# CAMMA-public/SelfPose3d

Measured on AMD Instinct MI355X. Metric: multi-view samples/sec (5-view Panoptic, 80x80x20 voxel), higher is better.
Workload: dtype f32

## Files before the change

selfpose3d_amd/build.py:

```python
from __future__ import annotations

import os
import subprocess
import sys

HERE = os.path.dirname(os.path.abspath(__file__))
CSRC = os.path.join(HERE, "csrc")
SOURCES = ["sp3d_unproject.hip", "sp3d_proposal.hip", "sp3d_epilogue.hip", "sp3d_upconv.hip", "sp3d_synth.hip", "sp3d_fftconv.hip", "sp3d_wino.hip",
           "sp3d_wino_fused.hip", "sp3d_conv3_direct.hip", "sp3d_fft.hip", "sp3d_gbn.hip"]
HEADERS = [os.path.join("..", "pk_src1.py"), "sp3d_conv3_host.h", "sp3d_device.h", "sp3d_proj_pk.h", "sp3d_split.h", "sp3d_tuning.h",
           "sp3d_twiddles.h", os.path.join("..", "..", "include", "sp3d.h")]
LIB = os.path.join(HERE, "libsp3d.so")
HIPCC = os.environ.get("HIPCC", "/opt/rocm/bin/hipcc")
FLAGS = ["--offload-arch=gfx950", "-O3", "-std=c++17", "-ffp-contract=off", "-munsafe-fp-atomics", "-fPIC", "-shared",
         "-Wall", "-Wno-unused-function"]
LINK = ["-L/opt/rocm/lib", "-lhipfft"]


def needs_build() -> bool:
    if not os.path.exists(LIB):
        return True
    t = os.path.getmtime(LIB)
    deps = [os.path.join(CSRC, s) for s in SOURCES + HEADERS] + [os.path.abspath(__file__)]
    return any(os.path.getmtime(d) > t for d in deps if os.path.exists(d))


PER_SOURCE_FLAGS = {"sp3d_wino.hip": ["-fno-slp-vectorize"], "sp3d_wino_fused.hip": ["-fno-slp-vectorize"],
                    "sp3d_conv3_direct.hip": ["-fno-slp-vectorize"], "sp3d_upconv.hip": ["-fno-slp-vectorize"],
                    "sp3d_fft.hip": ["-fno-slp-vectorize"], "sp3d_fftconv.hip": ["-fno-slp-vectorize"]}


LLVM_BIN = os.environ.get("SP3D_LLVM_BIN", "/opt/rocm/lib/llvm/bin")

NOPK_LIB = os.path.join(HERE, "libsp3d_nopk.so")
NOPK_FLAGS = ["-DSP3D_NO_PK", "-fno-slp-vectorize", "-Xclang", "-target-feature", "-Xclang", "-packed-fp32-ops"]




def _compile_one(src: str, objdir: str, cflags, verbose: bool, host_flags=()) -> str:
    from . import pk_src1
    base = os.path.join(objdir, src.replace(".hip", ""))
    path = os.path.join(CSRC, src)
    cuid = "-cuid=" + src.replace(".", "_")

    def run(cmd):
        if verbose:
            print(" ".join(cmd))
        subprocess.check_call(cmd)
    if os.environ.get("SP3D_PLAIN_HIPCC", "0") not in ("", "0"):
        flags = cflags + [f for f in NOPK_FLAGS if f not in cflags]
        run([HIPCC] + flags + ["-Wno-unused-command-line-argument", "-c", path, "-o", base + ".o"])
        return base + ".o"
    run([HIPCC] + cflags + ["-Wno-unused-command-line-argument", "--cuda-device-only", "-S", cuid, path, "-o", base + ".raw.s"])
    try:
        with open(base + ".raw.s") as fh:
            text, n = pk_src1.fix_asm(fh.read())
    except ValueError as e:
        import warnings
        warnings.warn(f"{src}: {e}; compiling this source without packed-fp32 instructions")
        cflags = cflags + [f for f in NOPK_FLAGS if f not in cflags]
        run([HIPCC] + cflags + ["-Wno-unused-command-line-argument", "--cuda-device-only", "-S", cuid, path, "-o", base + ".raw.s"])
        with open(base + ".raw.s") as fh:
            text, n = pk_src1.fix_asm(fh.read())
    if pk_src1.count_risky(text):
        raise RuntimeError(f"{src}: packed-fp32 instructions reading the high half of source 1 survive the rewrite")
    with open(base + ".s", "w") as fh:
        fh.write(text)
    os.remove(base + ".raw.s")
    if verbose:
        print(f"{src}: {n} packed-fp32 instructions rewritten (source 0 <-> source 1)")
    run([os.path.join(LLVM_BIN, "clang"), "-x", "assembler", "-target", "amdgcn-amd-amdhsa", "-mcpu=gfx950", "-c", base + ".s", "-o", base + ".dev.o"])
    run([os.path.join(LLVM_BIN, "lld"), "-flavor", "gnu", "-m", "elf64_amdgpu", "--no-undefined", "-shared", "-o", base + ".hsaco", base + ".dev.o"])
    run([os.path.join(LLVM_BIN, "clang-offload-bundler"), "-type=o", "-bundle-align=4096",
         "-targets=host-x86_64-unknown-linux-gnu,hipv4-amdgcn-amd-amdhsa--gfx950", "-input=/dev/null", "-input=" + base + ".hsaco",
         "-output=" + base + ".hipfb"])
    run([HIPCC] + cflags + list(host_flags) + ["-Wno-unused-command-line-argument", "--cuda-host-only", cuid, "-Xclang",
                                               "-fcuda-include-gpubinary", "-Xclang", base + ".hipfb", "-c", path, "-o", base + ".o"])
    for ext in (".dev.o", ".hsaco", ".hipfb"):
        os.remove(base + ext)
    return base + ".o"


def _compile_objects(objdir: str, extra_flags=(), verbose: bool = False, host_flags=()):
    from concurrent.futures import ThreadPoolExecutor
    os.makedirs(objdir, exist_ok=True)
    cflags = [f for f in FLAGS if f != "-shared"]
    with ThreadPoolExecutor(max_workers=len(SOURCES)) as pool:
        futs = [pool.submit(_compile_one, src, objdir, cflags + list(extra_flags) + PER_SOURCE_FLAGS.get(src, []), verbose, host_flags)
                for src in SOURCES]
        return [f.result() for f in futs]


def _link(objs, out: str, verbose: bool = False, link_flags=()):
    cmd = [HIPCC, "--offload-arch=gfx950", "-shared", "-fPIC"] + objs + LINK + list(link_flags) + ["-o", out]
    if verbose:
        print(" ".join(cmd))
    subprocess.check_call(cmd)


def build_variant(out: str, extra_flags=(), host_flags=(), link_flags=()) -> str:
    objdir = out + ".obj"
    _link(_compile_objects(objdir, extra_flags, host_flags=host_flags), out, link_flags=link_flags)
    return out


def _stale(lib: str) -> bool:
    if not os.path.exists(lib):
        return True
    t = os.path.getmtime(lib)
    deps = [os.path.join(CSRC, s) for s in SOURCES + HEADERS] + [os.path.abspath(__file__)]
    return any(os.path.getmtime(d) > t for d in deps if os.path.exists(d))


def build(force: bool = False, verbose: bool = False) -> str:
    if force or needs_build():
        objs = _compile_objects(os.path.join(HERE, "build", "obj"), verbose=verbose)
        _link(objs, LIB + ".tmp", verbose)
        os.replace(LIB + ".tmp", LIB)
    if force or _stale(NOPK_LIB):
        objs = _compile_objects(os.path.join(HERE, "build", "obj_nopk"), NOPK_FLAGS, verbose=verbose)
        _link(objs, NOPK_LIB + ".tmp", verbose)
        os.replace(NOPK_LIB + ".tmp", NOPK_LIB)
    return LIB


if __name__ == "__main__":
    print(build(force="--force" in sys.argv, verbose=True))
```

selfpose3d_amd/csrc/sp3d_conv3_direct.hip:

```cpp
#include <hip/hip_runtime.h>
#include <stdint.h>

#include "../../include/sp3d.h"
#include "sp3d_conv3_host.h"
#include "sp3d_split.h"

namespace sp3d {

constexpr int CD_BX = 16, CD_BY = 8, CD_BZ = 4;
constexpr int CD_RX = CD_BX + 2, CD_RY = CD_BY + 2, CD_RZ = CD_BZ + 2, CD_VOX = 8, CD_ROW = CD_RX * CD_VOX, CD_ZP = CD_RY * CD_ROW + 4;
constexpr int CD_PLANE = CD_RZ * CD_ZP;
constexpr int CD_BUF = 2 * CD_PLANE;
constexpr int CD_NV4 = CD_RX * CD_RY * CD_RZ * 2;
constexpr int CD_PROD = 4;
constexpr int CD_PER = (CD_NV4 + 64 * CD_PROD - 1) / (64 * CD_PROD);
constexpr int CD_BUFS = ((CD_BUF / 4 + 63) / 64) * 256;
#ifndef SP3D_WG_ABLATE
#define SP3D_WG_ABLATE 0
#endif
struct CdRec { u32x4 hl, hh, mm; };


#ifdef SP3D_CD_TIMELINE
__device__ unsigned long long *g_cd_tl = nullptr;
#define CD_STAMP(slot) do { __builtin_amdgcn_sched_barrier(0); if (g_cd_tl && blockIdx.x == 0 && lane == 0 && item < 64) { g_cd_tl[(wave * 64 + item) * 4 + (slot)] = __builtin_readcyclecounter(); \
     \
    if (wave == 0 && (slot) == 0 && item == 0) { g_cd_tl[(7 * 64 + 62) * 4 + 0] = wall_clock64(); g_cd_tl[(7 * 64 + 62) * 4 + 1] = __builtin_readcyclecounter(); } \
    if (wave == 0 && (slot) == 3) { g_cd_tl[(7 * 64 + 63) * 4 + 0] = wall_clock64(); g_cd_tl[(7 * 64 + 63) * 4 + 1] = __builtin_readcyclecounter(); } } __builtin_amdgcn_sched_barrier(0); } while (0)
#else
#define CD_STAMP(slot) do { (void)item; } while (0)
#endif

template <int C, int MODE, bool SKIP = false>
__global__ __launch_bounds__(64 * (4 + CD_PROD)) __attribute__((amdgpu_waves_per_eu(2, 2)))
void conv3_split_kernel(const float *__restrict__ x, const unsigned *__restrict__ W3, float *__restrict__ y,
                        const float *__restrict__ shift, const float *__restrict__ res, int B, int X, int Y, int Z, int NBX,
                        int NBY, int NBZ, int nblocks, const float *__restrict__ xs = nullptr,
                        const unsigned *__restrict__ WS = nullptr)
{
    constexpr int O = 32, NCH = C / 8, CS = 16;
    extern __shared__ __attribute__((aligned(16))) unsigned cd_lds[];
    const int tid = threadIdx.x, lane = tid & 63, wave = tid >> 6, t = lane & 31, h = lane >> 5;
    const int my_blocks = ((int)blockIdx.x < nblocks) ? (nblocks - 1 - (int)blockIdx.x) / (int)gridDim.x + 1 : 0;
    const int n_items = my_blocks * NCH;
    auto decode = [&](int item, int &b, int &ox0, int &oy0, int &oz0) {
        int bid = (int)blockIdx.x + (item / NCH) * (int)gridDim.x;
        const int bz = bid % NBZ; bid /= NBZ;
        const int by = bid % NBY; bid /= NBY;
        const int bx = bid % NBX;
        b = bid / NBX;
        ox0 = bx * CD_BX; oy0 = by * CD_BY; oz0 = bz * CD_BZ;
    };

    if (wave >= 4) {
        const int pt = tid - 256;
        __builtin_amdgcn_s_setprio(2);
        float4 d[CD_PER];
        int lo_[CD_PER], rel[CD_PER], vxyz[CD_PER];
#pragma unroll
        for (int u = 0; u < CD_PER; ++u) {
            const int idx = pt + 64 * CD_PROD * u;
            const int v = idx >> 1, half = idx & 1;
            const int vx = v % CD_RX, vy = (v / CD_RX) % CD_RY, vz = v / (CD_RX * CD_RY);
            lo_[u] = idx < CD_NV4 ? half * CD_PLANE + vz * CD_ZP + vy * CD_ROW + vx * CD_VOX : -1;
            rel[u] = ((vx * Y + vy) * Z + vz) * C + half * 4;
            vxyz[u] = idx < CD_NV4 ? (vx | (vy << 8) | (vz << 16)) : 0x00ffffff;
        }
        auto issue = [&](int k) {
            int b, ox0, oy0, oz0;
            decode(k, b, ox0, oy0, oz0);
            const int64_t vox0 = (((int64_t)b * X + (ox0 - 1)) * Y + (oy0 - 1)) * Z + (oz0 - 1);
            const float *xb = x + vox0 * C + (k % NCH) * 8;
            const int xlo = 1 - ox0, xhi = X + 1 - ox0, ylo = 1 - oy0, yhi = Y + 1 - oy0, zlo = 1 - oz0, zhi = Z + 1 - oz0;
#pragma unroll
            for (int u = 0; u < CD_PER; ++u) {
                const int vx = vxyz[u] & 255, vy = (vxyz[u] >> 8) & 255, vz = vxyz[u] >> 16;
                const bool in = vx >= xlo && vx < xhi && vy >= ylo && vy < yhi && vz >= zlo && vz < zhi;
                d[u] = make_float4(0.0f, 0.0f, 0.0f, 0.0f);
                if (in) d[u] = *reinterpret_cast<const float4 *>(xb + rel[u]);
            }
        };
        if (n_items > 0) issue(0);
        for (int k = 0; k <= n_items; ++k) {
            if (k < n_items) {
                { const int item = k; CD_STAMP(0); }
                unsigned *buf = cd_lds + (k & 1) * CD_BUFS;
#ifdef SP3D_CD_TIMELINE
                __builtin_amdgcn_s_waitcnt(0);
                { const int item = k; CD_STAMP(3); }
#endif
#pragma unroll
                for (int u = 0; u < CD_PER; ++u) {
                    u32x4 q0, q1;
                    split3(d[u], q0, q1);
                    if (lo_[u] >= 0) {
                        unsigned *p = buf + lo_[u];
                        *reinterpret_cast<u32x4 *>(p) = q0;
                        *reinterpret_cast<u32x4 *>(p + 4) = q1;
                    }
                }
                { const int item = k; CD_STAMP(1); }
                if (k + 1 < n_items) issue(k + 1);
            }
            if (k < n_items) { const int item = k; CD_STAMP(2); }
            __syncthreads();
        }
        return;
    }

    const int a_off = h * CD_PLANE + (t >> 3) * CD_ZP + (t & 7) * CD_ROW + 4 * wave * CD_VOX;
    const unsigned *wl = W3 + ((int64_t)h * O + t) * 12;
    struct W3Rec { CdRec d[3]; };
    auto load_w = [&](int q) {
        const int cc = (q / 9) % NCH, st = q % 9;
        const unsigned *r = wl + ((int64_t)(3 * st) * NCH + cc) * 2 * O * 12;
        W3Rec w;
#pragma unroll
        for (int dx = 0; dx < 3; ++dx) {
#if SP3D_W16_ABLATE & 2
            (void)r; w.d[dx].hl = u32x4{0x3f803f80u + (unsigned)q, 0x3f803f80u, 0x3f803f80u + (unsigned)dx, 0x3f803f80u};
            w.d[dx].hh = w.d[dx].hl ^ 0x00010001u; w.d[dx].mm = w.d[dx].hl ^ 0x00020002u;
#else
            w.d[dx].hl = *reinterpret_cast<const u32x4 *>(r + (int64_t)dx * NCH * 2 * O * 12);
            w.d[dx].hh = *reinterpret_cast<const u32x4 *>(r + (int64_t)dx * NCH * 2 * O * 12 + 4);
            w.d[dx].mm = *reinterpret_cast<const u32x4 *>(r + (int64_t)dx * NCH * 2 * O * 12 + 8);
#endif
        }
        return w;
    };
    struct Opnd { u32x4 lh[6], hm[6]; };
    f32x16 acc[4];
    W3Rec w0, w1;
    if (n_items > 0) w0 = load_w(0);
    __syncthreads();
    for (int k = 1; k <= n_items; ++k) {
        const int item = k - 1, cc = item % NCH;
        const unsigned *ab = cd_lds + (item & 1) * CD_BUFS + a_off;
        if (cc == 0) {
#pragma unroll
            for (int m = 0; m < 4; ++m)
#pragma unroll
                for (int v = 0; v < 16; ++v) acc[m][v] = 0.0f;
        }
        auto load_a = [&](int st, Opnd &a) {
            const int dz = st / 3, dy = st % 3;
#pragma unroll
            for (int j = 0; j < 6; ++j) {
                const unsigned *p = ab + dz * CD_ZP + dy * CD_ROW + j * CD_VOX;
                a.lh[j] = *reinterpret_cast<const u32x4 *>(p);
                a.hm[j] = *reinterpret_cast<const u32x4 *>(p + 4);
            }
        };
        Opnd a0, a1;
        load_a(0, a0);
        const int q0 = item * 9;
        float s0[4];
        unsigned so[4];
        CD_STAMP(0);
#pragma unroll
        for (int st = 0; st < 9; ++st) {
            if (SKIP && st == 8 && cc == NCH - 1) {
                int b, ox0, oy0, oz0;
                decode(item, b, ox0, oy0, oz0);
                const float *xb = xs + (int64_t)b * X * Y * Z * CS;
                const int ys = min(oy0 + (t & 7), Y - 1), zs = min(oz0 + (t >> 3), Z - 1);
#pragma unroll
                for (int i = 0; i < 4; ++i) {
                    const int xv = min(ox0 + 4 * wave + i, X - 1);
                    so[i] = (unsigned)(((xv * Y + ys) * Z + zs) * CS + 4 * h);
                    s0[i] = xb[so[i]];
                }
            }
            __builtin_amdgcn_sched_barrier(0);
            w1 = load_w(min(q0 + st + 1, n_items * 9 - 1));
            if (st + 1 < 9) load_a(st + 1, a1);
#pragma unroll
            for (int dx = 0; dx < 3; ++dx) {
#pragma unroll
                for (int i = 0; i < 4; ++i) acc[i] = mfma_bf16(a0.lh[i + dx], w0.d[dx].hl, acc[i]);
#pragma unroll
                for (int i = 0; i < 4; ++i) acc[i] = mfma_bf16(a0.hm[i + dx], w0.d[dx].hh, acc[i]);
#pragma unroll
                for (int i = 0; i < 4; ++i) acc[i] = mfma_bf16(a0.hm[i + dx], w0.d[dx].mm, acc[i]);
            }
#pragma unroll
            for (int r = 0; r < 12; ++r) {
                __builtin_amdgcn_sched_group_barrier(0x008, 1, 0);
                __builtin_amdgcn_sched_group_barrier(0x100, 1, 0);
            }
#pragma unroll
            for (int r = 0; r < 9; ++r) {
                __builtin_amdgcn_sched_group_barrier(0x008, 1, 0);
                __builtin_amdgcn_sched_group_barrier(0x020, 1, 0);
            }
            __builtin_amdgcn_sched_group_barrier(0x008, 15, 0);
            __builtin_amdgcn_sched_barrier(0);
            a0 = a1;
            w0 = w1;
        }
        CD_STAMP(1);
        if (SKIP && cc == NCH - 1) {
            float4 sv[2][4];
            {
                int b, ox0, oy0, oz0;
                decode(item, b, ox0, oy0, oz0);
                const float *xb = xs + (int64_t)b * X * Y * Z * CS;
#pragma unroll
                for (int i = 0; i < 4; ++i) {
                    const float *p = xb + so[i];
                    sv[0][i] = make_float4(s0[i], p[1], p[2], p[3]);
                    sv[1][i] = *reinterpret_cast<const float4 *>(p + 8);
                }
            }
            CdRec ws[2];
#pragma unroll
            for (int c2 = 0; c2 < 2; ++c2) {
                const unsigned *r = WS + (unsigned)(((c2 * 2 + h) * O + t) * 12);
                ws[c2].hl = *reinterpret_cast<const u32x4 *>(r);
                ws[c2].hh = *reinterpret_cast<const u32x4 *>(r + 4);
                ws[c2].mm = *reinterpret_cast<const u32x4 *>(r + 8);
            }
#pragma unroll
            for (int c2 = 0; c2 < 2; ++c2) {
                __builtin_amdgcn_sched_barrier(0);
                u32x4 lh[4], hm[4];
#pragma unroll
                for (int i = 0; i < 4; ++i) split3(sv[c2][i], lh[i], hm[i]);
#pragma unroll
                for (int i = 0; i < 4; ++i) acc[i] = mfma_bf16(lh[i], ws[c2].hl, acc[i]);
#pragma unroll
                for (int i = 0; i < 4; ++i) acc[i] = mfma_bf16(hm[i], ws[c2].hh, acc[i]);
#pragma unroll
                for (int i = 0; i < 4; ++i) acc[i] = mfma_bf16(hm[i], ws[c2].mm, acc[i]);
            }
        }
        if (cc == NCH - 1) {
            int b, ox0, oy0, oz0;
            decode(item, b, ox0, oy0, oz0);
            if (ox0 + CD_BX <= X && oy0 + CD_BY <= Y && oz0 + CD_BZ <= Z) {
                const float sh = shift[t];
                const int64_t obase = ((((int64_t)b * X + ox0 + 4 * wave) * Y + oy0 + 4 * h) * Z + oz0) * O + t;
#pragma unroll
                for (int i = 0; i < 4; ++i)
#pragma unroll
                    for (int v = 0; v < 16; ++v) {
                        const int64_t idx = obase + (((int64_t)i * Y + (v & 3)) * Z + (v >> 2)) * O;
                        float val = acc[i][v] + sh;
                        if (MODE == 2) val += res[idx];
                        if (MODE >= 1) val = SKIP ? relu_keep_nan(val) : fmaxf(val, 0.0f);
                        if (MODE == 3) val += res[idx];
#if SP3D_W16_ABLATE & 16
                        if (val == 123.456f)
#endif
                        y[idx] = val;
                    }
            } else {
            float *scr = reinterpret_cast<float *>(cd_lds + 2 * CD_BUFS) + wave * 1024;
            const int g = lane & 7;
            const float4 sh4 = *reinterpret_cast<const float4 *>(shift + 4 * g);
#pragma unroll
            for (int mb = 0; mb < 4; ++mb) {
#pragma unroll
                for (int v = 0; v < 16; ++v) scr[(8 * (v >> 2) + (v & 3) + 4 * h) * 32 + t] = acc[mb][v];
                __builtin_amdgcn_fence(__ATOMIC_RELEASE, "wavefront");
                __builtin_amdgcn_wave_barrier();
#pragma unroll
                for (int r = 0; r < 4; ++r) {
                    const int m = (lane >> 3) + 8 * r;
                    float4 a = *reinterpret_cast<const float4 *>(scr + m * 32 + 4 * g);
                    const int xo = ox0 + 4 * wave + mb, yo = oy0 + (m & 7), zo = oz0 + (m >> 3);
                    if (xo < X && yo < Y && zo < Z) {
                        const int64_t vox = (((int64_t)b * X + xo) * Y + yo) * Z + zo;
                        a.x += sh4.x; a.y += sh4.y; a.z += sh4.z; a.w += sh4.w;
                        float4 rr = make_float4(0.0f, 0.0f, 0.0f, 0.0f);
                        if (MODE >= 2) rr = *reinterpret_cast<const float4 *>(res + vox * O + 4 * g);
                        if (MODE == 2) { a.x += rr.x; a.y += rr.y; a.z += rr.z; a.w += rr.w; }
                        if (MODE >= 1 && SKIP) { a.x = relu_keep_nan(a.x); a.y = relu_keep_nan(a.y); a.z = relu_keep_nan(a.z); a.w = relu_keep_nan(a.w); }
                        if (MODE >= 1 && !SKIP) { a.x = fmaxf(a.x, 0.0f); a.y = fmaxf(a.y, 0.0f); a.z = fmaxf(a.z, 0.0f); a.w = fmaxf(a.w, 0.0f); }
                        if (MODE == 3) { a.x += rr.x; a.y += rr.y; a.z += rr.z; a.w += rr.w; }
#if SP3D_W16_ABLATE & 16
                        if (a.x == 123.456f)
#endif
                        *reinterpret_cast<float4 *>(y + vox * O + 4 * g) = a;
                    }
                }
                __builtin_amdgcn_fence(__ATOMIC_RELEASE, "wavefront");
                __builtin_amdgcn_wave_barrier();
            }
            }
        }
        CD_STAMP(2);
        __syncthreads();
        CD_STAMP(3);
    }
}


}


using namespace sp3d;

static int conv3_cu_count(int dev)
{
    static int cu_count[64] = {0};
    if (dev < 0 || dev >= 64) return 256;
    if (cu_count[dev] == 0) {
        int n = 0;
        cu_count[dev] = (hipDeviceGetAttribute(&n, hipDeviceAttributeMultiprocessorCount, dev) == hipSuccess && n > 0) ? n : 256;
    }
    return cu_count[dev];
}

template <int C, int MODE, bool SKIP>
static int conv3_split_launch(const float *x, const void *W3, float *y, const float *shift, const float *residual, const float *xs,
                              const void *WS, int B, int X, int Y, int Z, const Conv3Grid &g, void *stream)
{
    int dev = 0;
    { const hipError_t ed = hipGetDevice(&dev); if (ed != hipSuccess) return (int)ed; }
    const int cus = conv3_cu_count(dev);
    const int rounds = (int)((g.blocks + cus - 1) / cus);
    const int nwg = (int)((g.blocks + rounds - 1) / rounds);
    const size_t lds = (size_t)2 * CD_BUFS * sizeof(unsigned) + 4 * 1024 * sizeof(float);
    static bool attr_dev[64] = {};
    const int slot = (dev < 0 || dev >= 64) ? 63 : dev;
    if (!attr_dev[slot] || slot == 63) {
        const hipError_t ea = hipFuncSetAttribute(reinterpret_cast<const void *>(conv3_split_kernel<C, MODE, SKIP>),
                                                  hipFuncAttributeMaxDynamicSharedMemorySize, (int)lds);
        if (ea != hipSuccess) return (int)ea;
        attr_dev[slot] = true;
    }
    hipLaunchKernelGGL((conv3_split_kernel<C, MODE, SKIP>), dim3((unsigned)nwg), dim3(64 * (4 + CD_PROD)), lds, (hipStream_t)stream, x,
                       reinterpret_cast<const unsigned *>(W3), y, shift, residual, B, X, Y, Z, g.NBX, g.NBY, g.NBZ, (int)g.blocks, xs,
                       reinterpret_cast<const unsigned *>(WS));
    return launch_status();
}

extern "C" int sp3d_conv3_split(const float *x, const void *W3, float *y, const float *shift, const float *residual, int mode,
                                int B, int X, int Y, int Z, int C, int O, void *stream)
{
    const Conv3Grid g = conv3_grid(B, X, Y, Z, CD_BX, CD_BY, CD_BZ);
    const bool supported = O == 32 && (C == 16 || C == 32) && !((reinterpret_cast<uintptr_t>(W3) | reinterpret_cast<uintptr_t>(y)) & 15);
    const bool in_range = (int64_t)X * Y * Z * C * 2 <= 0x7fffffff && g.blocks <= 0x7fffffff;
    if (const int rc = conv3_check(B, X, Y, Z, mode, x && W3 && y && shift && (mode < 2 || residual), supported, in_range)) return rc;
    return with_mode(mode, [&](auto m) {
        constexpr int M = decltype(m)::value;
        return C == 16 ? conv3_split_launch<16, M, false>(x, W3, y, shift, residual, nullptr, nullptr, B, X, Y, Z, g, stream)
                       : conv3_split_launch<32, M, false>(x, W3, y, shift, residual, nullptr, nullptr, B, X, Y, Z, g, stream);
    });
}

extern "C" int sp3d_conv3_split_skip(const float *x, const void *W3, float *y, const float *shift, const float *xs,
                                     const void *WS, int B, int X, int Y, int Z, int C, int O, int CS, void *stream)
{
    const Conv3Grid g = conv3_grid(B, X, Y, Z, CD_BX, CD_BY, CD_BZ);
    const bool supported = O == 32 && C == 32 && CS == 16 &&
                           !((reinterpret_cast<uintptr_t>(W3) | reinterpret_cast<uintptr_t>(WS) | reinterpret_cast<uintptr_t>(xs) |
                              reinterpret_cast<uintptr_t>(y)) & 15);
    const bool in_range = (int64_t)X * Y * Z * C * 2 <= 0x7fffffff && g.blocks <= 0x7fffffff;
    if (const int rc = conv3_check(B, X, Y, Z, 1, x && W3 && y && shift && xs && WS, supported, in_range)) return rc;
    return conv3_split_launch<32, 1, true>(x, W3, y, shift, nullptr, xs, WS, B, X, Y, Z, g, stream);
}


extern "C" int sp3d_debug_conv3_timeline(void *dev_buffer)
{
#ifdef SP3D_CD_TIMELINE
    unsigned long long *p = (unsigned long long *)dev_buffer;
    return (int)hipMemcpyToSymbol(HIP_SYMBOL(sp3d::g_cd_tl), &p, sizeof(p));
#else
    (void)dev_buffer;
    return SP3D_EUNSUPPORTED;
#endif
}
```

selfpose3d_amd/csrc/sp3d_fft.hip:

```cpp
#include <hip/hip_runtime.h>
#include <hipfft/hipfft.h>
#include <stdint.h>

#include <map>
#include <mutex>
#include <tuple>

#include "../../include/sp3d.h"
#include "sp3d_twiddles.h"

namespace {
using Key = std::tuple<int, uintptr_t, int, int, int, int, int>;
std::mutex g_mu;
std::map<Key, hipfftHandle> g_plans;

int get_plan(int inverse, int batch, int SX, int SY, int SZ, void *stream, hipfftHandle *out)
{
    int dev = 0;
    hipError_t e = hipGetDevice(&dev);
    if (e != hipSuccess) return (int)e;
    const Key k{dev, (uintptr_t)stream, inverse, batch, SX, SY, SZ};
    std::lock_guard<std::mutex> lock(g_mu);
    auto it = g_plans.find(k);
    if (it != g_plans.end()) {
        *out = it->second;
        return SP3D_OK;
    }
    hipStreamCaptureStatus cs = hipStreamCaptureStatusNone;
    if (stream && hipStreamIsCapturing((hipStream_t)stream, &cs) == hipSuccess && cs == hipStreamCaptureStatusActive) {
        for (auto &kv : g_plans) {
            const Key &o = kv.first;
            if (std::get<0>(o) == dev && std::get<2>(o) == inverse && std::get<3>(o) == batch && std::get<4>(o) == SX &&
                std::get<5>(o) == SY && std::get<6>(o) == SZ) {
                *out = kv.second;
                return SP3D_OK;
            }
        }
        return SP3D_EFFT;
    }
    hipfftHandle p;
    int n[3] = {SX, SY, SZ};
    const hipfftResult r = inverse == 2 ? hipfftPlanMany(&p, 2, n, nullptr, 1, 0, nullptr, 1, 0, HIPFFT_C2C, batch)
                                        : hipfftPlanMany(&p, 3, n, nullptr, 1, 0, nullptr, 1, 0, inverse ? HIPFFT_C2R : HIPFFT_R2C, batch);
    if (r != HIPFFT_SUCCESS) return SP3D_EFFT;
    g_plans.emplace(k, p);
    *out = p;
    return SP3D_OK;
}

int check_args(const void *a, const void *b, int batch, int SX, int SY, int SZ)
{
    if (batch <= 0 || SX <= 0 || SY <= 0 || SZ <= 0) return SP3D_EINVAL;
    if (!a || !b) return SP3D_ENULL;
    if ((int64_t)batch * SX * SY * SZ > (int64_t)1 << 40) return SP3D_ERANGE;
    return SP3D_OK;
}
}

extern "C" int sp3d_rfft3d(const float *in, float *out, int batch, int SX, int SY, int SZ, void *stream)
{
    int rc = check_args(in, out, batch, SX, SY, SZ);
    if (rc) return rc;
    hipfftHandle p;
    if ((rc = get_plan(0, batch, SX, SY, SZ, stream, &p))) return rc;
    std::lock_guard<std::mutex> lock(g_mu);
    if (hipfftSetStream(p, (hipStream_t)stream) != HIPFFT_SUCCESS) return SP3D_EFFT;
    if (hipfftExecR2C(p, const_cast<float *>(in), reinterpret_cast<hipfftComplex *>(out)) != HIPFFT_SUCCESS) return SP3D_EFFT;
    return SP3D_OK;
}

extern "C" int sp3d_irfft3d(float *in, float *out, int batch, int SX, int SY, int SZ, void *stream)
{
    int rc = check_args(in, out, batch, SX, SY, SZ);
    if (rc) return rc;
    hipfftHandle p;
    if ((rc = get_plan(1, batch, SX, SY, SZ, stream, &p))) return rc;
    std::lock_guard<std::mutex> lock(g_mu);
    if (hipfftSetStream(p, (hipStream_t)stream) != HIPFFT_SUCCESS) return SP3D_EFFT;
    if (hipfftExecC2R(p, reinterpret_cast<hipfftComplex *>(in), out) != HIPFFT_SUCCESS) return SP3D_EFFT;
    return SP3D_OK;
}

extern "C" int sp3d_cfft2d(float *data, int batch, int SX, int SY, int inverse, void *stream)
{
    int rc = check_args(data, data, batch, SX, SY, 1);
    if (rc) return rc;
    hipfftHandle p;
    if ((rc = get_plan(2, batch, SX, SY, 0, stream, &p))) return rc;
    std::lock_guard<std::mutex> lock(g_mu);
    if (hipfftSetStream(p, (hipStream_t)stream) != HIPFFT_SUCCESS) return SP3D_EFFT;
    hipfftComplex *d = reinterpret_cast<hipfftComplex *>(data);
    if (hipfftExecC2C(p, d, d, inverse ? HIPFFT_BACKWARD : HIPFFT_FORWARD) != HIPFFT_SUCCESS) return SP3D_EFFT;
    return SP3D_OK;
}

namespace sp3d {

constexpr int ZD_TY = 16;
template <int Z, int C> constexpr int zd_pitch() { return Z * C + 4; }

template <int Z, int SZ, int C>
__global__ __launch_bounds__(256) void zdft_fwd_cl_kernel(const float *__restrict__ x, float2 *__restrict__ out, int X, int Y,
                                                         int SX, int SY, int Cout)
{
    static_assert(C == 16 && (Z * C) % 4 == 0, "16 channels x 16 positions = 256 threads");
    constexpr int K = SZ / 2 + 1, P = zd_pitch<Z, C>();
    __shared__ __attribute__((aligned(16))) float tile[ZD_TY * P];
    const int plane = SX * SY;
    const int ntile = (plane + ZD_TY - 1) / ZD_TY;
    const int b = blockIdx.x / ntile;
    const int p0 = (blockIdx.x - b * ntile) * ZD_TY;
    const int t = threadIdx.x, yy = t & 15, c = ((t >> 6) << 2) + ((t >> 4) & 3);
    constexpr int R4 = Z * C / 4;
    for (int i = t; i < ZD_TY * R4; i += 256) {
        const int row = i / R4, rem = i - row * R4;
        const int p = p0 + row, px = p / SY, py = p - px * SY;
        float4 v = make_float4(0.0f, 0.0f, 0.0f, 0.0f);
        if (px < X && py < Y) v = reinterpret_cast<const float4 *>(x + ((((int64_t)b * X + px) * Y + py) * Z) * C)[rem];
        *reinterpret_cast<float4 *>(tile + row * P + 4 * rem) = v;
    }
    __syncthreads();
    const int p = p0 + yy, px = p / SY, py = p - px * SY;
    float re[K], im[K];
#pragma unroll
    for (int k = 0; k < K; ++k) { re[k] = 0.0f; im[k] = 0.0f; }
    if (px < X && py < Y && c < Cout) {
        float v[Z];
#pragma unroll
        for (int z = 0; z < Z; ++z) v[z] = tile[yy * P + z * C + c];
        zdft_real<Z, SZ>(v, re, im);
    }
    if (c < Cout && p < plane) {
        float2 *o = out + (((int64_t)b * Cout + c) * K) * plane + p;
#pragma unroll
        for (int k = 0; k < K; ++k) o[(int64_t)k * plane] = make_float2(re[k], im[k]);
    }
}

template <int Z, int SZ, int O>
__global__ __launch_bounds__(256) void zdft_inv_cl_kernel(const float2 *__restrict__ in, float *__restrict__ y,
                                                         const float *__restrict__ shift, int X, int Y, int SX, int SY,
                                                         int relu)
{
    static_assert(O == 16 && (Z * O) % 4 == 0, "16 channels x 16 rows = 256 threads");
    constexpr int K = SZ / 2 + 1, P = zd_pitch<Z, O>();
    constexpr Twiddles<SZ> tw{};
    __shared__ __attribute__((aligned(16))) float tile[ZD_TY * P];
    const int nyt = (Y + ZD_TY - 1) / ZD_TY;
    int r = blockIdx.x;
    const int yt = r % nyt; r /= nyt;
    const int xx = r % X;
    const int b = r / X;
    const int y0 = yt * ZD_TY;
    const int t = threadIdx.x, yy = t & 15, o = ((t >> 6) << 2) + ((t >> 4) & 3);
    const int ny = min(ZD_TY, Y - y0);
    if (yy < ny) {
        const float2 *p = in + ((((int64_t)b * O + o) * K) * SX + xx) * SY + y0 + yy;
        float2 f[K];
#pragma unroll
        for (int k = 0; k < K; ++k) f[k] = p[(int64_t)k * SX * SY];
        const float sh = shift[o];
#pragma unroll
        for (int z = 0; z < Z; ++z) {
            float acc = f[0].x;
            if (SZ % 2 == 0) acc = (z & 1) ? acc - f[K - 1].x : acc + f[K - 1].x;
            constexpr int KL = (SZ % 2 == 0) ? K - 1 : K;
#pragma unroll
            for (int k = 1; k < KL; ++k) {
                const int m = (k * z) % SZ;
                acc = fmaf(2.0f * tw.c[m], f[k].x, acc);
                acc = fmaf(-2.0f * tw.s[m], f[k].y, acc);
            }
            acc += sh;
            if (relu) acc = acc < 0.0f ? 0.0f : acc;
            tile[yy * P + z * O + o] = acc;
        }
    }
    __syncthreads();
    float4 *dst = reinterpret_cast<float4 *>(y + ((((int64_t)b * X + xx) * Y + y0) * Z) * O);
    constexpr int R4 = Z * O / 4;
    for (int i = t; i < ny * R4; i += 256) {
        const int row = i / R4, rem = i - row * R4;
        dst[i] = *reinterpret_cast<const float4 *>(tile + row * P + 4 * rem);
    }
}


constexpr int F88 = 88, F88_PITCH = 89, F88_NT = 512;

__device__ __forceinline__ float2 cadd(float2 a, float2 b) { return make_float2(a.x + b.x, a.y + b.y); }
__device__ __forceinline__ float2 csub(float2 a, float2 b) { return make_float2(a.x - b.x, a.y - b.y); }
__device__ __forceinline__ float2 cmul(float2 a, float2 b) { return make_float2(fmaf(a.x, b.x, -a.y * b.y), fmaf(a.x, b.y, a.y * b.x)); }
__device__ __forceinline__ float2 mul_mi(float2 a) { return make_float2(a.y, -a.x); }

template <bool COLS> __device__ __forceinline__ int f88_at(int line, int pos) { return COLS ? pos * F88_PITCH + line : line * F88_PITCH + pos; }

template <bool COLS>
__device__ __forceinline__ void f88_pass(float2 *pl, const float2 *tws, int tid, int nlines)
{
    constexpr Twiddles<11> t11{};
    for (int task = tid; task < nlines * 8; task += F88_NT) {
        const int line = task % nlines, n2 = task / nlines;
        float2 a[11];
#pragma unroll
        for (int n1 = 0; n1 < 11; ++n1) a[n1] = pl[f88_at<COLS>(line, 8 * n1 + n2)];
        float2 sm[5], df[5];
#pragma unroll
        for (int j = 0; j < 5; ++j) { sm[j] = cadd(a[j + 1], a[10 - j]); df[j] = csub(a[j + 1], a[10 - j]); }
        float2 out[11];
        out[0] = a[0];
#pragma unroll
        for (int j = 0; j < 5; ++j) out[0] = cadd(out[0], sm[j]);
#pragma unroll
        for (int k = 1; k <= 5; ++k) {
            float2 cpart = a[0], spart = make_float2(0.0f, 0.0f);
#pragma unroll
            for (int j = 1; j <= 5; ++j) {
                const int m = (j * k) % 11;
                cpart.x = fmaf(sm[j - 1].x, t11.c[m], cpart.x); cpart.y = fmaf(sm[j - 1].y, t11.c[m], cpart.y);
                spart.x = fmaf(df[j - 1].x, t11.s[m], spart.x); spart.y = fmaf(df[j - 1].y, t11.s[m], spart.y);
            }
            out[k] = make_float2(cpart.x + spart.y, cpart.y - spart.x);
            out[11 - k] = make_float2(cpart.x - spart.y, cpart.y + spart.x);
        }
        pl[f88_at<COLS>(line, n2)] = out[0];
#pragma unroll
        for (int k1 = 1; k1 < 11; ++k1)
            pl[f88_at<COLS>(line, 8 * k1 + n2)] = n2 == 0 ? out[k1] : cmul(out[k1], tws[n2 * k1]);
    }
    __syncthreads();
    float2 b[2][8];
    const float r = 0.70710678118654752440f;
#pragma unroll
    for (int u = 0; u < 2; ++u) {
        const int task = tid + u * F88_NT;
        if (task < nlines * 11) {
            const int line = task % nlines, k1 = task / nlines;
#pragma unroll
            for (int n2 = 0; n2 < 8; ++n2) b[u][n2] = pl[f88_at<COLS>(line, 8 * k1 + n2)];
        }
    }
    __syncthreads();
#pragma unroll
    for (int u = 0; u < 2; ++u) {
        const int task = tid + u * F88_NT;
        if (task < nlines * 11) {
            const int line = task % nlines, k1 = task / nlines;
            const float2 *q = b[u];
            const float2 u0 = cadd(q[0], q[4]), u1 = csub(q[0], q[4]), u2 = cadd(q[2], q[6]), u3 = mul_mi(csub(q[2], q[6]));
            const float2 u4 = cadd(q[1], q[5]), u5 = csub(q[1], q[5]), u6 = cadd(q[3], q[7]), u7 = mul_mi(csub(q[3], q[7]));
            const float2 v0 = cadd(u0, u2), v2 = csub(u0, u2), v1 = cadd(u1, u3), v3 = csub(u1, u3);
            const float2 v4 = cadd(u4, u6), v6 = csub(u4, u6), v5 = cadd(u5, u7), v7 = csub(u5, u7);
            const float2 w5 = make_float2(r * (v5.x + v5.y), r * (v5.y - v5.x));
            const float2 w6 = mul_mi(v6);
            const float2 w7 = make_float2(r * (v7.y - v7.x), -r * (v7.x + v7.y));
            pl[f88_at<COLS>(line, k1)] = cadd(v0, v4);
            pl[f88_at<COLS>(line, k1 + 11)] = cadd(v1, w5);
            pl[f88_at<COLS>(line, k1 + 22)] = cadd(v2, w6);
            pl[f88_at<COLS>(line, k1 + 33)] = cadd(v3, w7);
            pl[f88_at<COLS>(line, k1 + 44)] = csub(v0, v4);
            pl[f88_at<COLS>(line, k1 + 55)] = csub(v1, w5);
            pl[f88_at<COLS>(line, k1 + 66)] = csub(v2, w6);
            pl[f88_at<COLS>(line, k1 + 77)] = csub(v3, w7);
        }
    }
    __syncthreads();
}

__global__ __launch_bounds__(F88_NT) void cfft2d_88_kernel(float2 *__restrict__ data, int inverse, int rows_in, int rows_out,
                                                           const float2 *__restrict__ tiled, int nby)
{
    extern __shared__ float2 lds88[];
    float2 *pl = lds88, *tws = lds88 + F88 * F88_PITCH;
    constexpr Twiddles<88> t88{};
    const int tid = threadIdx.x;
    float2 *base = data + (int64_t)blockIdx.x * F88 * F88;
    if (tid < F88) tws[tid] = make_float2(t88.c[tid], -t88.s[tid]);
    if (tiled) {
        for (int i = tid; i < F88 * F88_PITCH; i += F88_NT) pl[i] = make_float2(0.0f, 0.0f);
        __syncthreads();
        const int ntile = (rows_in / 4) * nby;
        const float4 *src = reinterpret_cast<const float4 *>(tiled + (int64_t)blockIdx.x * ntile * 16);
        for (int i = tid; i < ntile * 8; i += F88_NT) {
            const int tile = i >> 3, w = i & 7;
            const int tx = tile / nby, ty = tile - tx * nby;
            const int rr = 4 * tx + (w >> 1), cc = 4 * ty + 2 * (w & 1);
            const float4 v = src[i];
            pl[rr * F88_PITCH + cc] = make_float2(v.x, v.y);
            pl[rr * F88_PITCH + cc + 1] = make_float2(v.z, v.w);
        }
    } else
    for (int i = tid; i < F88 * F88 / 2; i += F88_NT) {
        const int e = 2 * i, rr = e / F88, cc = e - rr * F88;
        float4 v = make_float4(0.0f, 0.0f, 0.0f, 0.0f);
        if (rr < rows_in) v = reinterpret_cast<const float4 *>(base)[i];
        if (inverse) { v.y = -v.y; v.w = -v.w; }
        pl[rr * F88_PITCH + cc] = make_float2(v.x, v.y);
        pl[rr * F88_PITCH + cc + 1] = make_float2(v.z, v.w);
    }
    __syncthreads();
    if (rows_out < F88) {
        f88_pass<true>(pl, tws, tid, F88);
        f88_pass<false>(pl, tws, tid, rows_out);
    } else {
        f88_pass<false>(pl, tws, tid, rows_in);
        f88_pass<true>(pl, tws, tid, F88);
    }
    for (int i = tid; i < rows_out * F88 / 2; i += F88_NT) {
        const int e = 2 * i, rr = e / F88, cc = e - rr * F88;
        const float2 p0 = pl[rr * F88_PITCH + cc], p1 = pl[rr * F88_PITCH + cc + 1];
        float4 v = make_float4(p0.x, p0.y, p1.x, p1.y);
        if (inverse) { v.y = -v.y; v.w = -v.w; }
        reinterpret_cast<float4 *>(base)[i] = v;
    }
}
}

extern "C" int sp3d_zdft_fwd_cl(const float *x, float *spec, int B, int C, int Cout, int X, int Y, int Z, int SX, int SY, int SZ,
                                void *stream)
{
    if (B <= 0 || C <= 0 || Cout <= 0 || Cout > C || X <= 0 || Y <= 0 || Z <= 0 || SX < X || SY < Y || SZ < Z) return SP3D_EINVAL;
    if (!x || !spec) return SP3D_ENULL;
    if (!(C == 16 && Z == 20 && SZ == 28) || (reinterpret_cast<uintptr_t>(x) & 15)) return SP3D_EUNSUPPORTED;
    const int64_t blocks = (int64_t)B * (((int64_t)SX * SY + sp3d::ZD_TY - 1) / sp3d::ZD_TY);
    if (blocks > 0x7fffffff) return SP3D_ERANGE;
    hipLaunchKernelGGL((sp3d::zdft_fwd_cl_kernel<20, 28, 16>), dim3((unsigned)blocks), dim3(256), 0, (hipStream_t)stream, x,
                       reinterpret_cast<float2 *>(spec), X, Y, SX, SY, Cout);
    const hipError_t e = hipGetLastError();
    return e == hipSuccess ? SP3D_OK : (int)e;
}

extern "C" int sp3d_zdft_inv_cl(const float *spec, float *y, const float *shift, int B, int O, int X, int Y, int Z, int SX, int SY,
                                int SZ, int relu, void *stream)
{
    if (B <= 0 || O <= 0 || X <= 0 || Y <= 0 || Z <= 0 || SX < X || SY < Y || SZ < Z) return SP3D_EINVAL;
    if (!spec || !y || !shift) return SP3D_ENULL;
    if (!(O == 16 && Z == 20 && SZ == 28) || (reinterpret_cast<uintptr_t>(y) & 15)) return SP3D_EUNSUPPORTED;
    const int64_t blocks = (int64_t)B * X * ((Y + sp3d::ZD_TY - 1) / sp3d::ZD_TY);
    if (blocks > 0x7fffffff) return SP3D_ERANGE;
    hipLaunchKernelGGL((sp3d::zdft_inv_cl_kernel<20, 28, 16>), dim3((unsigned)blocks), dim3(256), 0, (hipStream_t)stream,
                       reinterpret_cast<const float2 *>(spec), y, shift, X, Y, SX, SY, relu);
    const hipError_t e = hipGetLastError();
    return e == hipSuccess ? SP3D_OK : (int)e;
}

static int f88_lds(size_t *bytes)
{
    *bytes = (size_t)(sp3d::F88 * sp3d::F88_PITCH + sp3d::F88) * sizeof(float2);
    static bool attr_set = false;
    if (!attr_set) {
        const hipError_t ea = hipFuncSetAttribute(reinterpret_cast<const void *>(sp3d::cfft2d_88_kernel),
                                                  hipFuncAttributeMaxDynamicSharedMemorySize, (int)*bytes);
        if (ea != hipSuccess) return (int)ea;
        attr_set = true;
    }
    return SP3D_OK;
}

extern "C" int sp3d_cfft2d_ex(float *data, int batch, int SX, int SY, int inverse, int rows_in, int rows_out, void *stream)
{
    if (batch <= 0 || SX <= 0 || SY <= 0 || rows_in <= 0 || rows_out <= 0 || rows_in > SX || rows_out > SX) return SP3D_EINVAL;
    if (!data) return SP3D_ENULL;
    if (SX != sp3d::F88 || SY != sp3d::F88 || (reinterpret_cast<uintptr_t>(data) & 15))
        return sp3d_cfft2d(data, batch, SX, SY, inverse, stream);
    size_t lds;
    if (const int ra = f88_lds(&lds)) return ra;
    hipLaunchKernelGGL(sp3d::cfft2d_88_kernel, dim3((unsigned)batch), dim3(sp3d::F88_NT), lds, (hipStream_t)stream,
                       reinterpret_cast<float2 *>(data), inverse, rows_in, rows_out, (const float2 *)nullptr, 0);
    const hipError_t e = hipGetLastError();
    return e == hipSuccess ? SP3D_OK : (int)e;
}

extern "C" int sp3d_cfft2d_88_tiled(const float *tiled, float *planes, int batch, int X, int Y, void *stream)
{
    if (batch <= 0 || X <= 0 || Y <= 0) return SP3D_EINVAL;
    if (!tiled || !planes) return SP3D_ENULL;
    if ((X & 3) || (Y & 3) || X > sp3d::F88 || Y > sp3d::F88 || (reinterpret_cast<uintptr_t>(tiled) & 15) ||
        (reinterpret_cast<uintptr_t>(planes) & 15))
        return SP3D_EUNSUPPORTED;
    size_t lds;
    if (const int ra = f88_lds(&lds)) return ra;
    hipLaunchKernelGGL(sp3d::cfft2d_88_kernel, dim3((unsigned)batch), dim3(sp3d::F88_NT), lds, (hipStream_t)stream,
                       reinterpret_cast<float2 *>(planes), 0, X, sp3d::F88, reinterpret_cast<const float2 *>(tiled), Y / 4);
    const hipError_t e = hipGetLastError();
    return e == hipSuccess ? SP3D_OK : (int)e;
}
```

Before: 2695.

## Make 88x88 FFT kernel persistent with register prefetch of next plane

Turns the 88x88 2D FFT kernel into a persistent kernel launched with about two workgroups per CU. Each workgroup loops over planes and prefetches the next plane's input into registers while the current plane is transformed. It also splits the kernel into tiled and untiled template variants and precomputes the load addressing. CU-count and LDS-attribute helpers move into a shared header. The goal is to hide global load latency and cut per-block launch overhead, at the cost of more registers and a grid-stride loop that may lower occupancy.

```diff
diff --git a/selfpose3d_amd/build.py b/selfpose3d_amd/build.py
--- a/selfpose3d_amd/build.py
+++ b/selfpose3d_amd/build.py
@@ -8,7 +8,7 @@
 CSRC = os.path.join(HERE, "csrc")
 SOURCES = ["sp3d_unproject.hip", "sp3d_proposal.hip", "sp3d_epilogue.hip", "sp3d_upconv.hip", "sp3d_synth.hip", "sp3d_fftconv.hip", "sp3d_wino.hip",
            "sp3d_wino_fused.hip", "sp3d_conv3_direct.hip", "sp3d_fft.hip", "sp3d_gbn.hip"]
-HEADERS = [os.path.join("..", "pk_src1.py"), "sp3d_conv3_host.h", "sp3d_device.h", "sp3d_proj_pk.h", "sp3d_split.h", "sp3d_tuning.h",
+HEADERS = [os.path.join("..", "pk_src1.py"), "sp3d_conv3_host.h", "sp3d_device.h", "sp3d_launch.h", "sp3d_proj_pk.h", "sp3d_split.h", "sp3d_tuning.h",
            "sp3d_twiddles.h", os.path.join("..", "..", "include", "sp3d.h")]
 LIB = os.path.join(HERE, "libsp3d.so")
 HIPCC = os.environ.get("HIPCC", "/opt/rocm/bin/hipcc")
diff --git a/selfpose3d_amd/csrc/sp3d_conv3_direct.hip b/selfpose3d_amd/csrc/sp3d_conv3_direct.hip
--- a/selfpose3d_amd/csrc/sp3d_conv3_direct.hip
+++ b/selfpose3d_amd/csrc/sp3d_conv3_direct.hip
@@ -3,6 +3,7 @@
 
 #include "../../include/sp3d.h"
 #include "sp3d_conv3_host.h"
+#include "sp3d_launch.h"
 #include "sp3d_split.h"
 
 namespace sp3d {
@@ -301,35 +302,19 @@
 
 using namespace sp3d;
 
-static int conv3_cu_count(int dev)
-{
-    static int cu_count[64] = {0};
-    if (dev < 0 || dev >= 64) return 256;
-    if (cu_count[dev] == 0) {
-        int n = 0;
-        cu_count[dev] = (hipDeviceGetAttribute(&n, hipDeviceAttributeMultiprocessorCount, dev) == hipSuccess && n > 0) ? n : 256;
-    }
-    return cu_count[dev];
-}
-
 template <int C, int MODE, bool SKIP>
 static int conv3_split_launch(const float *x, const void *W3, float *y, const float *shift, const float *residual, const float *xs,
                               const void *WS, int B, int X, int Y, int Z, const Conv3Grid &g, void *stream)
 {
     int dev = 0;
     { const hipError_t ed = hipGetDevice(&dev); if (ed != hipSuccess) return (int)ed; }
-    const int cus = conv3_cu_count(dev);
+    const int cus = device_cu_count(dev);
     const int rounds = (int)((g.blocks + cus - 1) / cus);
     const int nwg = (int)((g.blocks + rounds - 1) / rounds);
     const size_t lds = (size_t)2 * CD_BUFS * sizeof(unsigned) + 4 * 1024 * sizeof(float);
-    static bool attr_dev[64] = {};
-    const int slot = (dev < 0 || dev >= 64) ? 63 : dev;
-    if (!attr_dev[slot] || slot == 63) {
-        const hipError_t ea = hipFuncSetAttribute(reinterpret_cast<const void *>(conv3_split_kernel<C, MODE, SKIP>),
-                                                  hipFuncAttributeMaxDynamicSharedMemorySize, (int)lds);
-        if (ea != hipSuccess) return (int)ea;
-        attr_dev[slot] = true;
-    }
+    static bool attr_dev[MAX_DEV_SLOTS] = {};
+    if (const hipError_t ea = set_dynamic_lds_once(reinterpret_cast<const void *>(conv3_split_kernel<C, MODE, SKIP>), lds, dev, attr_dev))
+        return (int)ea;
     hipLaunchKernelGGL((conv3_split_kernel<C, MODE, SKIP>), dim3((unsigned)nwg), dim3(64 * (4 + CD_PROD)), lds, (hipStream_t)stream, x,
                        reinterpret_cast<const unsigned *>(W3), y, shift, residual, B, X, Y, Z, g.NBX, g.NBY, g.NBZ, (int)g.blocks, xs,
                        reinterpret_cast<const unsigned *>(WS));
diff --git a/selfpose3d_amd/csrc/sp3d_fft.hip b/selfpose3d_amd/csrc/sp3d_fft.hip
--- a/selfpose3d_amd/csrc/sp3d_fft.hip
+++ b/selfpose3d_amd/csrc/sp3d_fft.hip
@@ -7,6 +7,7 @@
 #include <tuple>
 
 #include "../../include/sp3d.h"
+#include "sp3d_launch.h"
 #include "sp3d_twiddles.h"
 
 namespace {
@@ -186,7 +187,14 @@
 }
 
 
-constexpr int F88 = 88, F88_PITCH = 89, F88_NT = 512;
+#ifndef SP3D_F88_NT
+#define SP3D_F88_NT 512
+#endif
+#ifndef SP3D_F88_PERSISTENT
+#define SP3D_F88_PERSISTENT 1
+#endif
+constexpr int F88 = 88, F88_PITCH = 89, F88_NT = SP3D_F88_NT;
+constexpr int F88_WAVES = 2 * F88_NT / 256;
 
 __device__ __forceinline__ float2 cadd(float2 a, float2 b) { return make_float2(a.x + b.x, a.y + b.y); }
 __device__ __forceinline__ float2 csub(float2 a, float2 b) { return make_float2(a.x - b.x, a.y - b.y); }
@@ -229,10 +237,11 @@
             pl[f88_at<COLS>(line, 8 * k1 + n2)] = n2 == 0 ? out[k1] : cmul(out[k1], tws[n2 * k1]);
     }
     __syncthreads();
-    float2 b[2][8];
+    constexpr int NB = (F88 * 11 + F88_NT - 1) / F88_NT;
+    float2 b[NB][8];
     const float r = 0.70710678118654752440f;
 #pragma unroll
-    for (int u = 0; u < 2; ++u) {
+    for (int u = 0; u < NB; ++u) {
         const int task = tid + u * F88_NT;
         if (task < nlines * 11) {
             const int line = task % nlines, k1 = task / nlines;
@@ -242,7 +251,7 @@
     }
     __syncthreads();
 #pragma unroll
-    for (int u = 0; u < 2; ++u) {
+    for (int u = 0; u < NB; ++u) {
         const int task = tid + u * F88_NT;
         if (task < nlines * 11) {
             const int line = task % nlines, k1 = task / nlines;
@@ -267,51 +276,95 @@
     __syncthreads();
 }
 
-__global__ __launch_bounds__(F88_NT) void cfft2d_88_kernel(float2 *__restrict__ data, int inverse, int rows_in, int rows_out,
-                                                           const float2 *__restrict__ tiled, int nby)
+constexpr int F88_NLD = (F88 * F88 / 2 + F88_NT - 1) / F88_NT;
+
+template <bool TILED>
+__global__ __launch_bounds__(F88_NT, F88_WAVES) void cfft2d_88_kernel(float2 *__restrict__ data, int inverse, int rows_in, int rows_out,
+                                                           const float2 *__restrict__ tiled, int nby, int batch)
 {
     extern __shared__ float2 lds88[];
     float2 *pl = lds88, *tws = lds88 + F88 * F88_PITCH;
     constexpr Twiddles<88> t88{};
     const int tid = threadIdx.x;
-    float2 *base = data + (int64_t)blockIdx.x * F88 * F88;
     if (tid < F88) tws[tid] = make_float2(t88.c[tid], -t88.s[tid]);
-    if (tiled) {
-        for (int i = tid; i < F88 * F88_PITCH; i += F88_NT) pl[i] = make_float2(0.0f, 0.0f);
+    const int nsig = TILED ? (rows_in / 4) * nby * 8 : rows_in * (F88 / 2);
+    const int nslot = TILED ? nsig : F88 * F88 / 2;
+    const int per_row = TILED ? nby : F88 / 2;
+    const int adv = TILED ? F88_NT / 8 : F88_NT;
+    const int adv_q = adv / per_row, adv_r = adv - adv_q * per_row;
+    int col0, off0, step, wrap;
+    if (TILED) {
+        const int tile = tid >> 3, w = tid & 7, tx = tile / nby;
+        col0 = tile - tx * nby;
+        off0 = (4 * tx + (w >> 1)) * F88_PITCH + 4 * col0 + 2 * (w & 1);
+        step = 4 * adv_q * F88_PITCH + 4 * adv_r; wrap = 4 * F88_PITCH - 4 * nby;
+    } else {
+        const int rr = tid / (F88 / 2);
+        col0 = tid - rr * (F88 / 2);
+        off0 = rr * F88_PITCH + 2 * col0;
+        step = adv_q * F88_PITCH + 2 * adv_r; wrap = F88_PITCH - F88;
+    }
+    const int64_t src_plane = TILED ? (int64_t)nsig * 2 : (int64_t)F88 * F88;
+    const float2 *src = TILED ? tiled : data;
+    float4 r[F88_NLD];
+    int p = blockIdx.x;
+    if (p >= batch) return;
+    {
+        const float4 *s4 = reinterpret_cast<const float4 *>(src + (int64_t)p * src_plane);
+#pragma unroll
+        for (int u = 0; u < F88_NLD; ++u) r[u] = s4[min(tid + u * F88_NT, nsig - 1)];
+    }
+    for (; p < batch; p += gridDim.x) {
+        float2 *base = data + (int64_t)p * F88 * F88;
+        if (TILED) {
+            for (int i = tid; i < F88 * F88 / 2; i += F88_NT) {
+                const int e = 2 * i, rr = e / F88, cc = e - rr * F88;
+                if (rr >= rows_in || cc >= 4 * nby) {
+                    pl[rr * F88_PITCH + cc] = make_float2(0.0f, 0.0f);
+                    pl[rr * F88_PITCH + cc + 1] = make_float2(0.0f, 0.0f);
+                }
+            }
+        }
+        int col = col0, off = off0;
+#pragma unroll
+        for (int u = 0; u < F88_NLD; ++u) {
+            const int i = tid + u * F88_NT;
+            if (i < nslot) {
+                float4 v = r[u];
+                if (!TILED) {
+                    if (i >= nsig) v = make_float4(0.0f, 0.0f, 0.0f, 0.0f);
+                    if (inverse) { v.y = -v.y; v.w = -v.w; }
+                }
+                pl[off] = make_float2(v.x, v.y);
+                pl[off + 1] = make_float2(v.z, v.w);
+            }
+            col += adv_r; off += step;
+            if (col >= per_row) { col -= per_row; off += wrap; }
+        }
+        if (SP3D_F88_PERSISTENT && p + (int)gridDim.x < batch) {
+            const float4 *s4 = reinterpret_cast<const float4 *>(src + (int64_t)(p + (int)gridDim.x) * src_plane);
+#pragma unroll
+            for (int u = 0; u < F88_NLD; ++u) r[u] = s4[min(tid + u * F88_NT, nsig - 1)];
+        }
         __syncthreads();
-        const int ntile = (rows_in / 4) * nby;
-        const float4 *src = reinterpret_cast<const float4 *>(tiled + (int64_t)blockIdx.x * ntile * 16);
-        for (int i = tid; i < ntile * 8; i += F88_NT) {
-            const int tile = i >> 3, w = i & 7;
-            const int tx = tile / nby, ty = tile - tx * nby;
-            const int rr = 4 * tx + (w >> 1), cc = 4 * ty + 2 * (w & 1);
-            const float4 v = src[i];
-            pl[rr * F88_PITCH + cc] = make_float2(v.x, v.y);
-            pl[rr * F88_PITCH + cc + 1] = make_float2(v.z, v.w);
-        }
-    } else
-    for (int i = tid; i < F88 * F88 / 2; i += F88_NT) {
-        const int e = 2 * i, rr = e / F88, cc = e - rr * F88;
-        float4 v = make_float4(0.0f, 0.0f, 0.0f, 0.0f);
-        if (rr < rows_in) v = reinterpret_cast<const float4 *>(base)[i];
-        if (inverse) { v.y = -v.y; v.w = -v.w; }
-        pl[rr * F88_PITCH + cc] = make_float2(v.x, v.y);
-        pl[rr * F88_PITCH + cc + 1] = make_float2(v.z, v.w);
-    }
-    __syncthreads();
-    if (rows_out < F88) {
-        f88_pass<true>(pl, tws, tid, F88);
-        f88_pass<false>(pl, tws, tid, rows_out);
-    } else {
-        f88_pass<false>(pl, tws, tid, rows_in);
-        f88_pass<true>(pl, tws, tid, F88);
-    }
-    for (int i = tid; i < rows_out * F88 / 2; i += F88_NT) {
-        const int e = 2 * i, rr = e / F88, cc = e - rr * F88;
-        const float2 p0 = pl[rr * F88_PITCH + cc], p1 = pl[rr * F88_PITCH + cc + 1];
-        float4 v = make_float4(p0.x, p0.y, p1.x, p1.y);
-        if (inverse) { v.y = -v.y; v.w = -v.w; }
-        reinterpret_cast<float4 *>(base)[i] = v;
+        int t = tid;
+        asm volatile("" : "+v"(t));
+        if (rows_out < F88) {
+            f88_pass<true>(pl, tws, t, F88);
+            f88_pass<false>(pl, tws, t, rows_out);
+        } else {
+            f88_pass<false>(pl, tws, t, rows_in);
+            f88_pass<true>(pl, tws, t, F88);
+        }
+        for (int i = t; i < rows_out * F88 / 2; i += F88_NT) {
+            const int e = 2 * i, rr = e / F88, cc = e - rr * F88;
+            const float2 p0 = pl[rr * F88_PITCH + cc], p1 = pl[rr * F88_PITCH + cc + 1];
+            float4 v = make_float4(p0.x, p0.y, p1.x, p1.y);
+            if (inverse) { v.y = -v.y; v.w = -v.w; }
+            reinterpret_cast<float4 *>(base)[i] = v;
+        }
+        if (!SP3D_F88_PERSISTENT) break;
+        __syncthreads();
     }
 }
 }
@@ -344,17 +397,21 @@
     return e == hipSuccess ? SP3D_OK : (int)e;
 }
 
-static int f88_lds(size_t *bytes)
-{
-    *bytes = (size_t)(sp3d::F88 * sp3d::F88_PITCH + sp3d::F88) * sizeof(float2);
-    static bool attr_set = false;
-    if (!attr_set) {
-        const hipError_t ea = hipFuncSetAttribute(reinterpret_cast<const void *>(sp3d::cfft2d_88_kernel),
-                                                  hipFuncAttributeMaxDynamicSharedMemorySize, (int)*bytes);
-        if (ea != hipSuccess) return (int)ea;
-        attr_set = true;
-    }
-    return SP3D_OK;
+template <bool TILED>
+static int f88_launch(float2 *data, int inverse, int rows_in, int rows_out, const float2 *tiled, int nby, int batch, void *stream)
+{
+    int dev = 0;
+    { const hipError_t ed = hipGetDevice(&dev); if (ed != hipSuccess) return (int)ed; }
+    const size_t lds = (size_t)(sp3d::F88 * sp3d::F88_PITCH + sp3d::F88) * sizeof(float2);
+    static bool attr_dev[sp3d::MAX_DEV_SLOTS] = {};
+    if (const hipError_t ea = sp3d::set_dynamic_lds_once(reinterpret_cast<const void *>(sp3d::cfft2d_88_kernel<TILED>), lds, dev, attr_dev))
+        return (int)ea;
+    const int slots = 2 * sp3d::device_cu_count(dev);
+    const int nwg = SP3D_F88_PERSISTENT ? (batch < slots ? batch : slots) : batch;
+    hipLaunchKernelGGL(sp3d::cfft2d_88_kernel<TILED>, dim3((unsigned)nwg), dim3(sp3d::F88_NT), lds, (hipStream_t)stream, data, inverse,
+                       rows_in, rows_out, tiled, nby, batch);
+    const hipError_t e = hipGetLastError();
+    return e == hipSuccess ? SP3D_OK : (int)e;
 }
 
 extern "C" int sp3d_cfft2d_ex(float *data, int batch, int SX, int SY, int inverse, int rows_in, int rows_out, void *stream)
@@ -363,12 +420,7 @@
     if (!data) return SP3D_ENULL;
     if (SX != sp3d::F88 || SY != sp3d::F88 || (reinterpret_cast<uintptr_t>(data) & 15))
         return sp3d_cfft2d(data, batch, SX, SY, inverse, stream);
-    size_t lds;
-    if (const int ra = f88_lds(&lds)) return ra;
-    hipLaunchKernelGGL(sp3d::cfft2d_88_kernel, dim3((unsigned)batch), dim3(sp3d::F88_NT), lds, (hipStream_t)stream,
-                       reinterpret_cast<float2 *>(data), inverse, rows_in, rows_out, (const float2 *)nullptr, 0);
-    const hipError_t e = hipGetLastError();
-    return e == hipSuccess ? SP3D_OK : (int)e;
+    return f88_launch<false>(reinterpret_cast<float2 *>(data), inverse, rows_in, rows_out, nullptr, 0, batch, stream);
 }
 
 extern "C" int sp3d_cfft2d_88_tiled(const float *tiled, float *planes, int batch, int X, int Y, void *stream)
@@ -378,10 +430,6 @@
     if ((X & 3) || (Y & 3) || X > sp3d::F88 || Y > sp3d::F88 || (reinterpret_cast<uintptr_t>(tiled) & 15) ||
         (reinterpret_cast<uintptr_t>(planes) & 15))
         return SP3D_EUNSUPPORTED;
-    size_t lds;
-    if (const int ra = f88_lds(&lds)) return ra;
-    hipLaunchKernelGGL(sp3d::cfft2d_88_kernel, dim3((unsigned)batch), dim3(sp3d::F88_NT), lds, (hipStream_t)stream,
-                       reinterpret_cast<float2 *>(planes), 0, X, sp3d::F88, reinterpret_cast<const float2 *>(tiled), Y / 4);
-    const hipError_t e = hipGetLastError();
-    return e == hipSuccess ? SP3D_OK : (int)e;
-}
+    return f88_launch<true>(reinterpret_cast<float2 *>(planes), 0, X, sp3d::F88, reinterpret_cast<const float2 *>(tiled), Y / 4, batch,
+                            stream);
+}
diff --git a/selfpose3d_amd/csrc/sp3d_launch.h b/selfpose3d_amd/csrc/sp3d_launch.h
--- /dev/null
+++ b/selfpose3d_amd/csrc/sp3d_launch.h
@@ -0,0 +1,32 @@
+#ifndef SP3D_LAUNCH_H
+#define SP3D_LAUNCH_H
+#include <hip/hip_runtime.h>
+
+namespace sp3d {
+
+constexpr int MAX_DEV_SLOTS = 64;
+
+inline int device_cu_count(int dev)
+{
+    static int cu_count[MAX_DEV_SLOTS] = {0};
+    if (dev < 0 || dev >= MAX_DEV_SLOTS) return 256;
+    if (cu_count[dev] == 0) {
+        int n = 0;
+        cu_count[dev] = (hipDeviceGetAttribute(&n, hipDeviceAttributeMultiprocessorCount, dev) == hipSuccess && n > 0) ? n : 256;
+    }
+    return cu_count[dev];
+}
+
+inline hipError_t set_dynamic_lds_once(const void *kernel, size_t bytes, int dev, bool *done)
+{
+    const int slot = (dev < 0 || dev >= MAX_DEV_SLOTS) ? MAX_DEV_SLOTS - 1 : dev;
+    if (!done[slot] || slot == MAX_DEV_SLOTS - 1) {
+        const hipError_t ea = hipFuncSetAttribute(kernel, hipFuncAttributeMaxDynamicSharedMemorySize, (int)bytes);
+        if (ea != hipSuccess) return ea;
+        done[slot] = true;
+    }
+    return hipSuccess;
+}
+
+}
+#endif
```

New measurement: 2703 (median of 4 runs). Within noise of the previous version (+0.3%).
